# nihaomiao/CVPR23_LFDM

Measured on AMD Instinct MI355X. Metric: 40-frame 128x128 videos/sec (DDIM-100), higher is better.
Workload: dtype f32; 1 GPU; MUG 128x128, 40-frame DDIM-100 sample, batch=1 per GPU (BASELINE.json configs[1]); global_batch=1, frames=40, latent=32, image=128, sampler=DDIM-100 eta=1, cond_scale=1, parallelism=replicas x1 (videos sharded, no collective)

## Files before the change

cvpr23_lfdm_amd/csrc/attention_fused.hip:

```cpp
#include <stdlib.h>

#include "attn_core.h"
#include "../../include/lfdm_hip.h"

namespace {

#ifdef LFDM_TATTN_STAMP
struct CycleProbe {
  long long t, acc[8];
  __device__ __forceinline__ void start() {
    for (int i = 0; i < 8; ++i) acc[i] = 0;
    t = clock64();
  }
  __device__ __forceinline__ void lap(int i) {
    LFDM_SCHED_FENCE();
    const long long now = clock64();
    acc[i] += now - t;
    t = now;
    LFDM_SCHED_FENCE();
  }
};
long long* tattn_stamps = nullptr;
#define TATTN_STAMP_PARAM , long long* stamps
#define TATTN_STAMP_ARG , tattn_stamps
#else
#define TATTN_STAMP_PARAM
#define TATTN_STAMP_ARG
#endif

template <int LP, int C, bool ROT_RELOAD = false, bool WPACK = false, bool PIPE = false, bool TO_LDS = false, class PROBE = NoProbe>
__device__ __forceinline__ void tattn_heads(const float* __restrict__ x, int ldx, int head_begin, int heads_per_block,
                                            const float* __restrict__ wqkv, float* __restrict__ out, int frames, int hw, int64_t seq,
                                            const float* __restrict__ bias, const float* __restrict__ rot_cos,
                                            const float* __restrict__ rot_sin, float eps, PROBE&& probe = NoProbe{}) {
  constexpr int NT = LP / 16;
  constexpr int CQ = C / 4;

  const int lane = threadIdx.x & 63;
  const int l15 = lane & 15, lq = lane >> 4;
  const int L = frames;
  const int64_t b = seq / hw, pix = seq - b * hw;
  const int64_t row0 = b * frames * hw + pix;

  float xf[NT][CQ];
#pragma unroll
  for (int ti = 0; ti < NT; ++ti) {
    const int t = ti * 16 + l15;
    float s1 = 0.f, s2 = 0.f;
    if (t < L) {
      const float* src = x + (row0 + (int64_t)t * hw) * ldx + CQ * lq;
#pragma unroll
      for (int q = 0; q < CQ / 4; ++q) {
        const float4 v = *reinterpret_cast<const float4*>(src + 4 * q);
        xf[ti][4 * q] = v.x; xf[ti][4 * q + 1] = v.y; xf[ti][4 * q + 2] = v.z; xf[ti][4 * q + 3] = v.w;
        ln_accum(v, s1, s2);
      }
    } else {
#pragma unroll
      for (int s = 0; s < CQ; ++s) xf[ti][s] = 0.f;
    }
    float mean, rstd;
    ln_stats_slots4<false>(s1, s2, C, eps, mean, rstd);
    if (t < L) {
#pragma unroll
      for (int s = 0; s < CQ; ++s) xf[ti][s] = (xf[ti][s] - mean) * rstd;
    }
  }

  float rc[NT][4], rs[NT][4];
  if (rot_cos && !ROT_RELOAD) {
#pragma unroll
    for (int ti = 0; ti < NT; ++ti) {
      const int t = ti * 16 + l15;
      const int tt = t < L ? t : 0;
#pragma unroll
      for (int fi = 0; fi < 2; ++fi)
#pragma unroll
        for (int pr = 0; pr < 2; ++pr) {
          rc[ti][2 * fi + pr] = rot_cos[tt * 16 + 8 * fi + 2 * lq + pr];
          rs[ti][2 * fi + pr] = rot_sin[tt * 16 + 8 * fi + 2 * lq + pr];
        }
    }
  }
  const bool bias_vec = bias && (L % 4 == 0) && ((((uintptr_t)bias) & 15) == 0);
  probe.lap(4);

#pragma unroll 1
  for (int head = head_begin; head < head_begin + heads_per_block; ++head) {
    float qf[NT][8], kf[NT][8];
    {
      float wa[4][CQ];
#pragma unroll
      for (int g = 0; g < 4; ++g) {
        const float* wsrc = WPACK ? wqkv + ((int64_t)(((g >> 1) * HEADS + head) * 2 + (g & 1)) * (CQ / 4) * 64 + lane) * 4
                                  : wqkv + ((int64_t)((g >> 1) * OUT_LD + head * DH + 16 * (g & 1) + l15)) * C + CQ * lq;
#pragma unroll
        for (int q = 0; q < CQ / 4; ++q) {
          const float4 v = *reinterpret_cast<const float4*>(wsrc + (WPACK ? 256 * q : 4 * q));
          wa[g][4 * q] = v.x; wa[g][4 * q + 1] = v.y; wa[g][4 * q + 2] = v.z; wa[g][4 * q + 3] = v.w;
        }
      }
#pragma unroll
      for (int g = 0; g < 4; ++g) {
        f32x4 acc[NT];
#pragma unroll
        for (int ti = 0; ti < NT; ++ti) acc[ti] = (f32x4){0.f, 0.f, 0.f, 0.f};
#pragma unroll
        for (int s = 0; s < CQ; ++s)
#pragma unroll
          for (int ti = 0; ti < NT; ++ti) acc[ti] = mfma_16x16x4(wa[g][s], xf[ti][s], acc[ti]);
#pragma unroll
        for (int ti = 0; ti < NT; ++ti)
#pragma unroll
          for (int r = 0; r < 4; ++r) {
            if ((g >> 1) == 0) qf[ti][4 * (g & 1) + r] = acc[ti][r] * ATT_SCALE;
            else kf[ti][4 * (g & 1) + r] = acc[ti][r];
          }
      }
    }
    if (rot_cos) {
#pragma unroll
      for (int ti = 0; ti < NT; ++ti) {
#pragma unroll
        for (int fi = 0; fi < 2; ++fi)
#pragma unroll
          for (int pr = 0; pr < 2; ++pr) {
            float c, sn;
            if (ROT_RELOAD) {
              const int t = ti * 16 + l15, tt = t < L ? t : 0;
              c = rot_cos[tt * 16 + 8 * fi + 2 * lq + pr];
              sn = rot_sin[tt * 16 + 8 * fi + 2 * lq + pr];
            } else {
              c = rc[ti][2 * fi + pr];
              sn = rs[ti][2 * fi + pr];
            }
            rot_pair(qf[ti][4 * fi + 2 * pr], qf[ti][4 * fi + 2 * pr + 1], c, sn);
            rot_pair(kf[ti][4 * fi + 2 * pr], kf[ti][4 * fi + 2 * pr + 1], c, sn);
          }
      }
    }
    float vf[2][4 * NT];
    {
      float wb[2][CQ];
#pragma unroll
      for (int half = 0; half < 2; ++half) {
        const float* wsrc = WPACK ? wqkv + ((int64_t)((2 * HEADS + head) * 2 + half) * (CQ / 4) * 64 + lane) * 4
                                  : wqkv + ((int64_t)(2 * OUT_LD + head * DH + 16 * half + l15)) * C + CQ * lq;
#pragma unroll
        for (int q = 0; q < CQ / 4; ++q) {
          const float4 v = *reinterpret_cast<const float4*>(wsrc + (WPACK ? 256 * q : 4 * q));
          wb[half][4 * q] = v.x; wb[half][4 * q + 1] = v.y; wb[half][4 * q + 2] = v.z; wb[half][4 * q + 3] = v.w;
        }
      }
#pragma unroll
      for (int half = 0; half < 2; ++half) {
        f32x4 acc[NT];
#pragma unroll
        for (int ti = 0; ti < NT; ++ti) acc[ti] = (f32x4){0.f, 0.f, 0.f, 0.f};
#pragma unroll
        for (int s = 0; s < CQ; ++s)
#pragma unroll
          for (int ti = 0; ti < NT; ++ti) acc[ti] = mfma_16x16x4(xf[ti][s], wb[half][s], acc[ti]);
#pragma unroll
        for (int ti = 0; ti < NT; ++ti)
#pragma unroll
          for (int r = 0; r < 4; ++r) vf[half][4 * ti + r] = acc[ti][r];
      }
    }

    probe.lap(0);
    attend_store<NT, false, PIPE, TO_LDS>(qf, kf, vf, head, L, l15, lq, bias, bias_vec, out, row0, hw, probe);
  }
}

template <int LP, int C, bool PIPE>
__global__ __launch_bounds__(64, 2) void temporal_attn_fused_kernel(const float* __restrict__ x, int ldx, int heads_per_block,
                                                                 const float* __restrict__ wqkv,
                                                                 float* __restrict__ out, int frames, int hw,
                                                                 const float* __restrict__ bias,
                                                                 const float* __restrict__ rot_cos,
                                                                 const float* __restrict__ rot_sin, float eps) {
  tattn_heads<LP, C, false, false, PIPE>(x, ldx, blockIdx.y * heads_per_block, heads_per_block, wqkv, out, frames, hw, blockIdx.x, bias, rot_cos, rot_sin, eps);
}

template <int LP, int LROWS, int NW, bool PIPE>
__global__ __launch_bounds__(64 * NW, 2) void temporal_attn_fused_out_kernel(const float* __restrict__ x, int ldx,
                                                                          const float* __restrict__ wqkv, const float* __restrict__ wout,
                                                                          float* __restrict__ out, int ldo, int frames, int hw,
                                                                          const float* __restrict__ bias, const float* __restrict__ rot_cos,
                                                                          const float* __restrict__ rot_sin, float eps TATTN_STAMP_PARAM) {
  constexpr int C = 64, NT = LP / 16, CT = C / 16;
  __shared__ __attribute__((aligned(16))) float o_lds[LROWS * OUT_LD];
  const int wave = lfdm_uniform((int)(threadIdx.x >> 6));
  const int lane = threadIdx.x & 63, l15 = lane & 15, lq = lane >> 4;
  const int L = frames;
  const int64_t seq = blockIdx.x;
#ifdef LFDM_TATTN_STAMP
  CycleProbe probe;
  probe.start();
#else
  NoProbe probe;
#endif
  tattn_heads<LP, C, (NW < 8), true, PIPE, true>(x, ldx, wave * (HEADS / NW), HEADS / NW, wqkv, o_lds, frames, hw, seq, bias, rot_cos, rot_sin, eps, probe);
  __syncthreads();
  probe.lap(5);
  const int64_t b = seq / hw, pix = seq - b * hw;
  const int64_t row0 = b * frames * hw + pix;
  for (int tile = wave; tile < NT * CT; tile += NW) {
    const int ti = tile / CT, ct = tile - ti * CT;
    const int t = ti * 16 + l15;
    const int tr = t < L ? t : L - 1;
    const float* arow = o_lds + tr * OUT_LD;
    const float* brow = wout + ((int64_t)ct * (OUT_LD / 16) * 64 + lane) * 4;
    f32x4 acc = {0.f, 0.f, 0.f, 0.f}, acc1 = acc;
    float xr[4];
#pragma unroll
    for (int r = 0; r < 4; ++r) {
      const int tok = ti * 16 + 4 * lq + r;
      xr[r] = x[(row0 + (int64_t)(tok < L ? tok : L - 1) * hw) * ldx + ct * 16 + l15];
    }
#pragma unroll 4
    for (int S = 0; S < OUT_LD / 16; S += 2) {
      const float4 a = *reinterpret_cast<const float4*>(arow + (((4 * S + lq) ^ (tr & 15)) << 2));
      const float4 a1 = *reinterpret_cast<const float4*>(arow + (((4 * S + 4 + lq) ^ (tr & 15)) << 2));
      const float4 w = *reinterpret_cast<const float4*>(brow + 256 * S);
      const float4 w1 = *reinterpret_cast<const float4*>(brow + 256 * S + 256);
      acc = mfma_16x16x4(a.x, w.x, acc);
      acc1 = mfma_16x16x4(a1.x, w1.x, acc1);
      acc = mfma_16x16x4(a.y, w.y, acc);
      acc1 = mfma_16x16x4(a1.y, w1.y, acc1);
      acc = mfma_16x16x4(a.z, w.z, acc);
      acc1 = mfma_16x16x4(a1.z, w1.z, acc1);
      acc = mfma_16x16x4(a.w, w.w, acc);
      acc1 = mfma_16x16x4(a1.w, w1.w, acc1);
    }
#pragma unroll
    for (int r = 0; r < 4; ++r) acc[r] += acc1[r];
#pragma unroll
    for (int r = 0; r < 4; ++r) {
      const int tok = ti * 16 + 4 * lq + r;
      if (tok < L) {
        const int64_t row = row0 + (int64_t)tok * hw;
        out[row * ldo + ct * 16 + l15] = acc[r] + xr[r];
      }
    }
  }
#ifdef LFDM_TATTN_STAMP
  probe.lap(6);
  if (stamps && lane == 0 && blockIdx.x < 256)
    for (int i = 0; i < 8; ++i) stamps[((int64_t)blockIdx.x * 8 + wave) * 8 + i] = probe.acc[i];
#endif
}

template <int LP, bool PIPE>
__global__ __launch_bounds__(64, 1) void temporal_attn_fused_wide_kernel(const float* __restrict__ x, int ldx, int channels,
                                                                      int heads_per_block, const float* __restrict__ wqkv,
                                                                      float* __restrict__ out, int frames, int hw,
                                                                      const float* __restrict__ bias,
                                                                      const float* __restrict__ rot_cos,
                                                                      const float* __restrict__ rot_sin, float eps) {
  constexpr int NT = LP / 16;
  const int lane = threadIdx.x & 63;
  const int l15 = lane & 15, lq = lane >> 4;
  const int L = frames;
  const int64_t seq = blockIdx.x;
  const int64_t b = seq / hw, pix = seq - b * hw;
  const int64_t row0 = b * frames * hw + pix;
  const int ncb = channels / 64;

  float mean[NT], rstd[NT];
#pragma unroll
  for (int ti = 0; ti < NT; ++ti) {
    const int t = ti * 16 + l15;
    float s1 = 0.f, s2 = 0.f;
    if (t < L) {
      const float* src = x + (row0 + (int64_t)t * hw) * ldx + 16 * lq;
      for (int cb = 0; cb < ncb; ++cb)
#pragma unroll
        for (int q = 0; q < 4; ++q) ln_accum(*reinterpret_cast<const float4*>(src + 64 * cb + 4 * q), s1, s2);
    }
    ln_stats_slots4<true>(s1, s2, channels, eps, mean[ti], rstd[ti]);
  }
  const bool bias_vec = bias && (L % 4 == 0) && ((((uintptr_t)bias) & 15) == 0);

  const int head_begin = blockIdx.y * heads_per_block;
#pragma unroll 1
  for (int head = head_begin; head < head_begin + heads_per_block; ++head) {
    f32x4 aq[2][NT], ak[2][NT], av[2][NT];
#pragma unroll
    for (int g = 0; g < 2; ++g)
#pragma unroll
      for (int ti = 0; ti < NT; ++ti) aq[g][ti] = ak[g][ti] = av[g][ti] = (f32x4){0.f, 0.f, 0.f, 0.f};
#pragma unroll 1
    for (int cb = 0; cb < ncb; ++cb) {
      float w[6][16];
#pragma unroll
      for (int g = 0; g < 6; ++g) {
        const float* wsrc = wqkv + ((int64_t)((g >> 1) * OUT_LD + head * DH + 16 * (g & 1) + l15)) * channels + 64 * cb + 16 * lq;
#pragma unroll
        for (int q = 0; q < 4; ++q) {
          const float4 v = *reinterpret_cast<const float4*>(wsrc + 4 * q);
          w[g][4 * q] = v.x; w[g][4 * q + 1] = v.y; w[g][4 * q + 2] = v.z; w[g][4 * q + 3] = v.w;
        }
      }
#pragma unroll
      for (int ti = 0; ti < NT; ++ti) {
        const int t = ti * 16 + l15;
        float xf[16];
        if (t < L) {
          const float* src = x + (row0 + (int64_t)t * hw) * ldx + 64 * cb + 16 * lq;
#pragma unroll
          for (int q = 0; q < 4; ++q) {
            const float4 v = *reinterpret_cast<const float4*>(src + 4 * q);
            xf[4 * q] = (v.x - mean[ti]) * rstd[ti]; xf[4 * q + 1] = (v.y - mean[ti]) * rstd[ti];
            xf[4 * q + 2] = (v.z - mean[ti]) * rstd[ti]; xf[4 * q + 3] = (v.w - mean[ti]) * rstd[ti];
          }
        } else {
#pragma unroll
          for (int s2 = 0; s2 < 16; ++s2) xf[s2] = 0.f;
        }
#pragma unroll
        for (int s2 = 0; s2 < 16; ++s2) {
          aq[0][ti] = mfma_16x16x4(w[0][s2], xf[s2], aq[0][ti]);
          aq[1][ti] = mfma_16x16x4(w[1][s2], xf[s2], aq[1][ti]);
          ak[0][ti] = mfma_16x16x4(w[2][s2], xf[s2], ak[0][ti]);
          ak[1][ti] = mfma_16x16x4(w[3][s2], xf[s2], ak[1][ti]);
          av[0][ti] = mfma_16x16x4(xf[s2], w[4][s2], av[0][ti]);
          av[1][ti] = mfma_16x16x4(xf[s2], w[5][s2], av[1][ti]);
        }
      }
    }
    float qf[NT][8], kf[NT][8], vf[2][4 * NT];
#pragma unroll
    for (int ti = 0; ti < NT; ++ti)
#pragma unroll
      for (int fi = 0; fi < 2; ++fi)
#pragma unroll
        for (int r = 0; r < 4; ++r) {
          qf[ti][4 * fi + r] = aq[fi][ti][r] * ATT_SCALE;
          kf[ti][4 * fi + r] = ak[fi][ti][r];
          vf[fi][4 * ti + r] = av[fi][ti][r];
        }
    if (rot_cos) {
#pragma unroll
      for (int ti = 0; ti < NT; ++ti) {
        const int t = ti * 16 + l15;
        const int tt = t < L ? t : 0;
#pragma unroll
        for (int fi = 0; fi < 2; ++fi)
#pragma unroll
          for (int pr = 0; pr < 2; ++pr) {
            const float c = rot_cos[tt * 16 + 8 * fi + 2 * lq + pr], sn = rot_sin[tt * 16 + 8 * fi + 2 * lq + pr];
            rot_pair(qf[ti][4 * fi + 2 * pr], qf[ti][4 * fi + 2 * pr + 1], c, sn);
            rot_pair(kf[ti][4 * fi + 2 * pr], kf[ti][4 * fi + 2 * pr + 1], c, sn);
          }
      }
    }
    attend_store<NT, false, PIPE>(qf, kf, vf, head, L, l15, lq, bias, bias_vec, out, row0, hw);
  }
}

int launch_fused_wide(const float* x, int ldx, int channels, const float* wqkv, float* out, int batch, int frames, int hw,
                      const float* bias, const float* rot_cos, const float* rot_sin, float eps, hipStream_t stream) {
  const int64_t nseq = (int64_t)batch * hw;
  int hpb = 8;
  while (hpb > 1 && nseq * (HEADS / hpb) < 2048) hpb >>= 1;
  const dim3 grid((unsigned)nseq, (unsigned)(HEADS / hpb)), block(64);
  lp_ladder(frames, [&](auto lp) {
    constexpr int LP = decltype(lp)::value;
    if (bias_by_quads(bias, frames))
      LFDM_LAUNCH((temporal_attn_fused_wide_kernel<LP, true>), grid, block, 0, stream, x, ldx, channels, hpb, wqkv, out, frames, hw, bias, rot_cos, rot_sin, eps);
    else
      LFDM_LAUNCH((temporal_attn_fused_wide_kernel<LP, false>), grid, block, 0, stream, x, ldx, channels, hpb, wqkv, out, frames, hw, bias, rot_cos, rot_sin, eps);
  });
  return lfdm_check_launch("temporal_attention_fused_wide");
}

template <int C>
int launch_fused(const float* x, int ldx, const float* wqkv, float* out, int batch, int frames, int hw, const float* bias,
                 const float* rot_cos, const float* rot_sin, float eps, hipStream_t stream) {
  const int64_t nseq = (int64_t)batch * hw;
  int hpb = 8;
  while (hpb > 1 && nseq * (HEADS / hpb) < 2048) hpb >>= 1;
  if (const char* e = lfdm_knob("LFDM_TATTN_HPB")) {
    const int v = atoi(e);
    if (v == 1 || v == 2 || v == 4 || v == 8) hpb = v;
  }
  const dim3 grid((unsigned)nseq, (unsigned)(HEADS / hpb)), block(64);
  lp_ladder(frames, [&](auto lp) {
    constexpr int LP = decltype(lp)::value;
    constexpr bool CAN_PIPE = LP <= 32;
    if (CAN_PIPE && bias_by_quads(bias, frames))
      LFDM_LAUNCH((temporal_attn_fused_kernel<LP, C, CAN_PIPE>), grid, block, 0, stream, x, ldx, hpb, wqkv, out, frames, hw, bias, rot_cos, rot_sin, eps);
    else
      LFDM_LAUNCH((temporal_attn_fused_kernel<LP, C, false>), grid, block, 0, stream, x, ldx, hpb, wqkv, out, frames, hw, bias, rot_cos, rot_sin, eps);
  });
  return lfdm_check_launch("temporal_attention_fused");
}

template <int LP, int LROWS>
int launch_fused_out_lp(const float* x, int ldx, const float* wqkv, const float* wout, float* out, int ldo, int batch, int frames, int hw,
                        const float* bias, const float* rot_cos, const float* rot_sin, float eps, hipStream_t stream) {
  const int64_t nseq = (int64_t)batch * hw;
  int nw = 2;
  while (nw < 8 && nseq * nw < 2048) nw <<= 1;
  if (const char* e = getenv("LFDM_TATTN_OUT_NW")) {
    const int v = atoi(e);
    if (v == 1 || v == 2 || v == 4 || v == 8) nw = v;
  }
  const dim3 grid((unsigned)nseq);
  lfdm_ladder<1, 2, 4, 8>(nw, [&](auto nwc) {
    constexpr int NW = decltype(nwc)::value;
#if defined(LFDM_TATTN_STAMP) && LFDM_TATTN_STAMP == 2
    constexpr bool CAN_PIPE = false;
#else
    constexpr bool CAN_PIPE = !(LP == 64 && NW == 4);
#endif
    if (CAN_PIPE && bias_by_quads(bias, frames))
      LFDM_LAUNCH((temporal_attn_fused_out_kernel<LP, LROWS, NW, CAN_PIPE>), grid, dim3(64 * NW), 0, stream, x, ldx, wqkv, wout, out, ldo, frames, hw, bias, rot_cos, rot_sin, eps TATTN_STAMP_ARG);
    else
      LFDM_LAUNCH((temporal_attn_fused_out_kernel<LP, LROWS, NW, false>), grid, dim3(64 * NW), 0, stream, x, ldx, wqkv, wout, out, ldo, frames, hw, bias, rot_cos, rot_sin, eps TATTN_STAMP_ARG);
  });
  return lfdm_check_launch("temporal_attention_fused_out");
}

}

#ifdef LFDM_TATTN_STAMP
extern "C" void lfdm_tattn_stamp_buffer(void* p) { tattn_stamps = (long long*)p; }
#endif

extern "C" int lfdm_temporal_attention_fused_out_cl_f32(const float* x, int ldx, int channels, const float* wqkv, const float* wout,
                                                        float* out, int ldo, int batch, int frames, int hw, const float* bias,
                                                        const float* rot_cos, const float* rot_sin, float ln_eps, lfdm_stream_t stream_) {
  hipStream_t stream = (hipStream_t)stream_;
  if (!x || !wqkv || !wout || !out || batch <= 0 || frames <= 0 || frames > 64 || hw <= 0 || channels != 64 || ldx < 64 || ldx % 4 != 0 ||
      ldo < 64 || (((uintptr_t)x | (uintptr_t)wqkv | (uintptr_t)wout) & 15) || ((rot_cos == nullptr) != (rot_sin == nullptr)) || out == x) {
    lfdm_set_error("temporal_attention_fused_out: needs C == 64, frames <= 64, 16-byte aligned rows, out != x");
    return LFDM_EINVAL;
  }
  return lp_ladder(frames, [&](auto lp) {
    constexpr int LP = decltype(lp)::value;
    if (LP == 48 && frames <= 40)
      return launch_fused_out_lp<48, 40>(x, ldx, wqkv, wout, out, ldo, batch, frames, hw, bias, rot_cos, rot_sin, ln_eps, stream);
    return launch_fused_out_lp<LP, LP>(x, ldx, wqkv, wout, out, ldo, batch, frames, hw, bias, rot_cos, rot_sin, ln_eps, stream);
  });
}

extern "C" int lfdm_temporal_attention_fused_cl_f32(const float* x, int ldx, int channels, const float* wqkv, float* out,
                                                    int batch, int frames, int hw, const float* bias,
                                                    const float* rot_cos, const float* rot_sin, float ln_eps,
                                                    lfdm_stream_t stream_) {
  hipStream_t stream = (hipStream_t)stream_;
  if (!x || !wqkv || !out || batch <= 0 || frames <= 0 || frames > 64 || hw <= 0 || ldx < channels || ldx % 4 != 0 ||
      (((uintptr_t)x | (uintptr_t)wqkv) & 15) || ((rot_cos == nullptr) != (rot_sin == nullptr)) ||
      channels < 64 || channels % 64 != 0) {
    lfdm_set_error("temporal_attention_fused: needs C % 64 == 0, frames <= 64, 16-byte aligned rows");
    return LFDM_EINVAL;
  }
  if (channels == 64) return launch_fused<64>(x, ldx, wqkv, out, batch, frames, hw, bias, rot_cos, rot_sin, ln_eps, stream);
  return launch_fused_wide(x, ldx, channels, wqkv, out, batch, frames, hw, bias, rot_cos, rot_sin, ln_eps, stream);
}
```

cvpr23_lfdm_amd/csrc/lfdm_device.h:

```cpp
#pragma once
#include <stddef.h>
#include <stdint.h>
#include <type_traits>

#if defined(LFDM_EMU_BUILD)
#include "hip_emu.h"
typedef emu_f32x16 f32x16;
typedef emu_f32x4 f32x4;
#define LFDM_LAUNCH(kern, grid, block, smem, stream, ...) \
  emu::launch(grid, block, smem, [=]() { kern(__VA_ARGS__); })
static inline f32x16 mfma_32x32x2(float a, float b, f32x16 c) { return emu_mfma_32x32x2(a, b, c); }
static inline f32x4 mfma_16x16x4(float a, float b, f32x4 c) { return emu_mfma_16x16x4(a, b, c); }
static inline f32x4 mfma_4x4x1(float a, float b, f32x4 c) { return emu_mfma_4x4x1(a, b, c); }
struct lfdm_bf16x8 { uint16_t h[8]; };
static inline uint16_t lfdm_f32_to_bf16(float f) {
  uint32_t u;
  memcpy(&u, &f, 4);
  if ((u & 0x7fffffffu) > 0x7f800000u) return (uint16_t)((u >> 16) | 0x40u);
  u += 0x7fffu + ((u >> 16) & 1u);
  return (uint16_t)(u >> 16);
}
static inline float lfdm_bf16_to_f32(uint16_t h) {
  const uint32_t u = (uint32_t)h << 16;
  float f;
  memcpy(&f, &u, 4);
  return f;
}
static inline lfdm_bf16x8 lfdm_cvt_bf16x8(float4 a0, float4 a1) {
  const float f[8] = {a0.x, a0.y, a0.z, a0.w, a1.x, a1.y, a1.z, a1.w};
  lfdm_bf16x8 r;
  for (int i = 0; i < 8; ++i) r.h[i] = lfdm_f32_to_bf16(f[i]);
  return r;
}
static inline uint32_t lfdm_cvt_pk_bf16(float lo, float hi) { return (uint32_t)lfdm_f32_to_bf16(lo) | ((uint32_t)lfdm_f32_to_bf16(hi) << 16); }
static inline lfdm_bf16x8 lfdm_bf16x8_bits(float4 v) {
  lfdm_bf16x8 r;
  memcpy(&r, &v, 16);
  return r;
}
static inline f32x16 mfma_32x32x16_bf16(lfdm_bf16x8 a, lfdm_bf16x8 b, f32x16 c) {
  struct Pair { lfdm_bf16x8 a, b; };
  struct Whole { lfdm_bf16x8 a[2], b[2]; };
  const unsigned lane = emu::lane_id(), h = lane >> 5;
  const Pair other = emu::wave_read_from(Pair{a, b}, lane ^ 32u);
  Whole mine;
  mine.a[h] = a;
  mine.a[1 - h] = other.a;
  mine.b[h] = b;
  mine.b[1 - h] = other.b;
  for (int r = 0; r < 16; ++r) {
    const unsigned row = (r & 3) + 8 * (r >> 2) + 4 * h;
    const Whole src = emu::wave_read_from(mine, row);
    float acc = c[r];
    for (int k = 0; k < 16; ++k)
      acc = fmaf(lfdm_bf16_to_f32(src.a[k >> 3].h[k & 7]), lfdm_bf16_to_f32(mine.b[k >> 3].h[k & 7]), acc);
    c[r] = acc;
  }
  return c;
}
#else
#include <hip/hip_runtime.h>
typedef float f32x16 __attribute__((ext_vector_type(16)));
typedef float f32x4 __attribute__((ext_vector_type(4)));
#define LFDM_LAUNCH(kern, grid, block, smem, stream, ...) \
  hipLaunchKernelGGL(kern, grid, block, smem, stream, __VA_ARGS__)
__device__ __forceinline__ f32x16 mfma_32x32x2(float a, float b, f32x16 c) {
  return __builtin_amdgcn_mfma_f32_32x32x2f32(a, b, c, 0, 0, 0);
}
__device__ __forceinline__ f32x4 mfma_16x16x4(float a, float b, f32x4 c) {
  return __builtin_amdgcn_mfma_f32_16x16x4f32(a, b, c, 0, 0, 0);
}
__device__ __forceinline__ f32x4 mfma_4x4x1(float a, float b, f32x4 c) {
  return __builtin_amdgcn_mfma_f32_4x4x1f32(a, b, c, 0, 0, 0);
}
typedef __bf16 lfdm_bf16x8 __attribute__((ext_vector_type(8)));
typedef __bf16 lfdm_bf16x2 __attribute__((ext_vector_type(2)));
typedef float lfdm_f32x8 __attribute__((ext_vector_type(8)));
typedef float lfdm_f32x2 __attribute__((ext_vector_type(2)));
__device__ __forceinline__ lfdm_bf16x8 lfdm_cvt_bf16x8(float4 a0, float4 a1) {
  const lfdm_f32x8 f = {a0.x, a0.y, a0.z, a0.w, a1.x, a1.y, a1.z, a1.w};
  return __builtin_convertvector(f, lfdm_bf16x8);
}
__device__ __forceinline__ uint32_t lfdm_cvt_pk_bf16(float lo, float hi) {
  const lfdm_f32x2 f = {lo, hi};
  return __builtin_bit_cast(uint32_t, __builtin_convertvector(f, lfdm_bf16x2));
}
__device__ __forceinline__ lfdm_bf16x8 lfdm_bf16x8_bits(float4 v) { return __builtin_bit_cast(lfdm_bf16x8, v); }
__device__ __forceinline__ f32x16 mfma_32x32x16_bf16(lfdm_bf16x8 a, lfdm_bf16x8 b, f32x16 c) {
  return __builtin_amdgcn_mfma_f32_32x32x16_bf16(a, b, c, 0, 0, 0);
}
#endif

#define LFDM_WAVE 64

template <int BEGIN, int END, class F>
__device__ __forceinline__ void lfdm_static_for(F&& f) {
  if constexpr (BEGIN < END) {
    f(std::integral_constant<int, BEGIN>{});
    lfdm_static_for<BEGIN + 1, END>(f);
  }
}

template <int R, int... REST, class F>
inline auto lfdm_ladder(int v, F&& f) {
  if constexpr (sizeof...(REST) == 0) return f(std::integral_constant<int, R>{});
  else return v <= R ? f(std::integral_constant<int, R>{}) : lfdm_ladder<REST...>(v, f);
}

#if defined(LFDM_EMU_BUILD)
struct lfdm_buf {
  const char* base;
  uint32_t bytes;
};
static inline lfdm_buf lfdm_make_buf(const void* p, uint32_t bytes) { return lfdm_buf{(const char*)p, bytes}; }
static inline float4 lfdm_buf_load_f4(lfdm_buf b, uint32_t off) {
  float4 v = make_float4(0.f, 0.f, 0.f, 0.f);
  if ((uint64_t)off + 16u <= (uint64_t)b.bytes) memcpy(&v, b.base + off, 16);
  return v;
}
static inline float2 lfdm_buf_load_f2(lfdm_buf b, uint32_t off) {
  float2 v = make_float2(0.f, 0.f);
  if ((uint64_t)off + 8u <= (uint64_t)b.bytes) memcpy(&v, b.base + off, 8);
  return v;
}
#else
typedef __amdgpu_buffer_rsrc_t lfdm_buf;
typedef int lfdm_i32x4 __attribute__((ext_vector_type(4)));
__device__ __forceinline__ lfdm_buf lfdm_make_buf(const void* p, uint32_t bytes) {
  return __builtin_amdgcn_make_buffer_rsrc(const_cast<void*>(p), 0, (int)bytes, 0x00020000);
}
__device__ __forceinline__ float4 lfdm_buf_load_f4(lfdm_buf b, uint32_t off) {
  const lfdm_i32x4 v = __builtin_amdgcn_raw_buffer_load_b128(b, (int)off, 0, 0);
  float4 f;
  f.x = __int_as_float(v.x);
  f.y = __int_as_float(v.y);
  f.z = __int_as_float(v.z);
  f.w = __int_as_float(v.w);
  return f;
}
typedef int lfdm_i32x2 __attribute__((ext_vector_type(2)));
__device__ __forceinline__ float2 lfdm_buf_load_f2(lfdm_buf b, uint32_t off) {
  const lfdm_i32x2 v = __builtin_amdgcn_raw_buffer_load_b64(b, (int)off, 0, 0);
  return make_float2(__int_as_float(v.x), __int_as_float(v.y));
}
#endif
#define LFDM_BUF_OOB 0xFFFFFFF0u

#if defined(LFDM_EMU_BUILD)
static inline void lfdm_buf_store_f4_sc1(lfdm_buf b, uint32_t off, float4 v) {
  if ((uint64_t)off + 16u <= (uint64_t)b.bytes) memcpy(const_cast<char*>(b.base) + off, &v, 16);
}
static inline float4 lfdm_buf_load_f4_sc1(lfdm_buf b, uint32_t off) { return lfdm_buf_load_f4(b, off); }
#else
__device__ __forceinline__ void lfdm_buf_store_f4_sc1(lfdm_buf b, uint32_t off, float4 v) {
  lfdm_i32x4 d;
  d.x = __float_as_int(v.x); d.y = __float_as_int(v.y); d.z = __float_as_int(v.z); d.w = __float_as_int(v.w);
  __builtin_amdgcn_raw_buffer_store_b128(d, b, (int)off, 0, 16);
}
__device__ __forceinline__ float4 lfdm_buf_load_f4_sc1(lfdm_buf b, uint32_t off) {
  const lfdm_i32x4 v = __builtin_amdgcn_raw_buffer_load_b128(b, (int)off, 0, 16);
  float4 f;
  f.x = __int_as_float(v.x); f.y = __int_as_float(v.y); f.z = __int_as_float(v.z); f.w = __int_as_float(v.w);
  return f;
}
#endif

#if defined(LFDM_EMU_BUILD)
template <int OFF = 0> static inline void lfdm_gload_f4(f32x4& dst, const float* p) { memcpy(&dst, (const char*)p + OFF, 16); }
template <int N> static inline void lfdm_vmwait() {}
template <int N> static inline void lfdm_vmwait(f32x4&) {}
template <int N> static inline void lfdm_vmwait(f32x4&, f32x4&) {}
template <int N> static inline void lfdm_vmwait(f32x4&, f32x4&, f32x4&, f32x4&) {}
static inline void lfdm_tie(f32x4&) {}
static inline int lfdm_uniform(int v) { return v; }
#else
template <int OFF = 0>
__device__ __forceinline__ void lfdm_gload_f4(f32x4& dst, const float* p) {
  asm volatile("global_load_dwordx4 %0, %1, off offset:%2" : "=v"(dst) : "v"(p), "n"(OFF) : "memory");
}
template <int N> __device__ __forceinline__ void lfdm_vmwait() { asm volatile("s_waitcnt vmcnt(%0)" ::"n"(N) : "memory"); }
template <int N> __device__ __forceinline__ void lfdm_vmwait(f32x4& a) { asm volatile("s_waitcnt vmcnt(%1)" : "+v"(a) : "n"(N) : "memory"); }
template <int N> __device__ __forceinline__ void lfdm_vmwait(f32x4& a, f32x4& b) {
  asm volatile("s_waitcnt vmcnt(%2)" : "+v"(a), "+v"(b) : "n"(N) : "memory");
}
template <int N> __device__ __forceinline__ void lfdm_vmwait(f32x4& a, f32x4& b, f32x4& c, f32x4& d) {
  asm volatile("s_waitcnt vmcnt(%4)" : "+v"(a), "+v"(b), "+v"(c), "+v"(d) : "n"(N) : "memory");
}
__device__ __forceinline__ void lfdm_tie(f32x4& a) { asm volatile("" : "+v"(a)::"memory"); }
__device__ __forceinline__ int lfdm_uniform(int v) { return __builtin_amdgcn_readfirstlane(v); }
#endif

#if defined(LFDM_EMU_BUILD)
#define LFDM_DRAIN_STORES() ((void)0)
#define LFDM_FENCE_RELEASE_AGENT() ((void)0)
#define LFDM_FENCE_ACQUIRE_AGENT() ((void)0)
static inline unsigned lfdm_ticket_take(unsigned* c) { return __atomic_fetch_add(c, 1u, __ATOMIC_SEQ_CST); }
static inline void lfdm_ticket_reset(unsigned* c) { __atomic_store_n(c, 0u, __ATOMIC_SEQ_CST); }
#else
#define LFDM_DRAIN_STORES() asm volatile("s_waitcnt vmcnt(0)" ::: "memory")
#define LFDM_FENCE_RELEASE_AGENT() __builtin_amdgcn_fence(__ATOMIC_RELEASE, "agent")
#define LFDM_FENCE_ACQUIRE_AGENT() __builtin_amdgcn_fence(__ATOMIC_ACQUIRE, "agent")
__device__ __forceinline__ unsigned lfdm_ticket_take(unsigned* c) {
  return __hip_atomic_fetch_add(c, 1u, __ATOMIC_RELAXED, __HIP_MEMORY_SCOPE_AGENT);
}
__device__ __forceinline__ void lfdm_ticket_reset(unsigned* c) {
  __hip_atomic_store(c, 0u, __ATOMIC_RELAXED, __HIP_MEMORY_SCOPE_AGENT);
}
#endif

#if defined(__HIP_DEVICE_COMPILE__) && !defined(__gfx950__) && !defined(LFDM_EMU_BUILD)
#error "fence-free hand-off (lfdm_agent_store_u64 / lfdm_agent_load_u64 / lfdm_ticket_take) validated on gfx950 only: re-validate, or use LFDM_FENCE_RELEASE_AGENT / LFDM_FENCE_ACQUIRE_AGENT, before building for another target"
#endif
#if defined(LFDM_EMU_BUILD)
static inline void lfdm_agent_store_u64(unsigned long long* p, unsigned long long v) { __atomic_store_n(p, v, __ATOMIC_SEQ_CST); }
static inline unsigned long long lfdm_agent_load_u64(const unsigned long long* p) { return __atomic_load_n(p, __ATOMIC_SEQ_CST); }
static inline unsigned lfdm_agent_load_u32(const unsigned* p) { return __atomic_load_n(p, __ATOMIC_SEQ_CST); }
static inline void lfdm_sleep() {}
#else
__device__ __forceinline__ void lfdm_agent_store_u64(unsigned long long* p, unsigned long long v) {
  __hip_atomic_store(p, v, __ATOMIC_RELAXED, __HIP_MEMORY_SCOPE_AGENT);
}
__device__ __forceinline__ unsigned long long lfdm_agent_load_u64(const unsigned long long* p) {
  return __hip_atomic_load(p, __ATOMIC_RELAXED, __HIP_MEMORY_SCOPE_AGENT);
}
__device__ __forceinline__ unsigned lfdm_agent_load_u32(const unsigned* p) { return __hip_atomic_load(p, __ATOMIC_RELAXED, __HIP_MEMORY_SCOPE_AGENT); }
__device__ __forceinline__ void lfdm_sleep() { __builtin_amdgcn_s_sleep(2); }
#endif

#if defined(LFDM_EMU_BUILD)
#define LFDM_SCHED_FENCE() ((void)0)
#define LFDM_SCHED_GROUP(mask, n) ((void)0)
#else
#define LFDM_SCHED_FENCE() __builtin_amdgcn_sched_barrier(0)
#define LFDM_SCHED_GROUP(mask, n) __builtin_amdgcn_sched_group_barrier(mask, n, 0)
#endif
#define LFDM_SG_VALU 0x002
#define LFDM_SG_MFMA 0x008

#if defined(LFDM_EMU_BUILD)
static inline void lfdm_wave_lds_sync() { emu::wave_sync(); }
#else
__device__ __forceinline__ void lfdm_wave_lds_sync() {
  __builtin_amdgcn_fence(__ATOMIC_RELEASE, "wavefront");
  __builtin_amdgcn_wave_barrier();
  __builtin_amdgcn_fence(__ATOMIC_ACQUIRE, "wavefront");
}
#endif

__device__ __forceinline__ float wave_sum(float v) {
#pragma unroll
  for (int m = 32; m >= 1; m >>= 1) v += __shfl_xor(v, m);
  return v;
}
__device__ __forceinline__ float wave_max(float v) {
#pragma unroll
  for (int m = 32; m >= 1; m >>= 1) v = fmaxf(v, __shfl_xor(v, m));
  return v;
}
#if defined(LFDM_EMU_BUILD)
static inline float fast_exp(float x) { return expf(x); }
static inline float fast_rcp(float x) { return 1.0f / x; }
#else
__device__ __forceinline__ float fast_exp(float x) { return __expf(x); }
__device__ __forceinline__ float fast_rcp(float x) { return __builtin_amdgcn_rcpf(x); }
#endif
__device__ __forceinline__ float sigmoidf_(float x) { return 1.0f / (1.0f + expf(-x)); }
__device__ __forceinline__ float siluf_(float x) { return x / (1.0f + expf(-x)); }

#if defined(LFDM_EMU_BUILD)
static inline float silu_fast_(float x) { return x / (1.0f + expf(-x)); }
#else
__device__ __forceinline__ float silu_fast_(float x) { return x * __builtin_amdgcn_rcpf(1.0f + __expf(-x)); }
#endif

#if defined(LFDM_TUNING_KNOBS) || defined(LFDM_EMU_BUILD)
static inline const char* lfdm_knob(const char* name) { return getenv(name); }
#else
static inline const char* lfdm_knob(const char*) { return nullptr; }
#endif

__device__ __forceinline__ float apply_act(float v, int act) {
  if (act == 1) return v > 0.f ? v : 0.f;
  if (act == 2) return sigmoidf_(v);
  if (act == 3) return siluf_(v);
  return v;
}

extern "C" void lfdm_set_error(const char* msg);
int lfdm_check_launch(const char* what);
```

Before: 4.180 videos/s.

## Restructure temporal attention out-projection with register weight ring and column-major wave mapping

The output projection in the fused temporal attention kernel is rewritten so each wave owns fixed output column tiles and handles several token tiles at once. The wout fragments are prefetched into a register ring before the barrier, overlapping global loads with the attention tail. LDS A-operands are double-buffered across steps. This reuses weights across token tiles and hides load latency, at the cost of higher register pressure that may hurt occupancy. Lane id is recomputed through mbcnt to keep it out of long-lived registers.

Result: no change. 4.201 videos/s (median of 6 runs) (+0.5%).

```diff
diff --git a/cvpr23_lfdm_amd/csrc/attention_fused.hip b/cvpr23_lfdm_amd/csrc/attention_fused.hip
--- a/cvpr23_lfdm_amd/csrc/attention_fused.hip
+++ b/cvpr23_lfdm_amd/csrc/attention_fused.hip
@@ -183,6 +183,94 @@
   tattn_heads<LP, C, false, false, PIPE>(x, ldx, blockIdx.y * heads_per_block, heads_per_block, wqkv, out, frames, hw, blockIdx.x, bias, rot_cos, rot_sin, eps);
 }
 
+template <int WD>
+__device__ __forceinline__ float4 wout_fragment(const float* __restrict__ wout, int ct0, int ctstep, int p, int lane) {
+  const float* frag = wout + (int64_t)((ct0 + (p >> 4) * ctstep) * (OUT_LD / 16) + (p & 15)) * 256;
+  return *reinterpret_cast<const float4*>(frag + 4 * lane);
+}
+template <int WD>
+__device__ __forceinline__ void wout_ring_fill(float4 (&w)[WD], const float* __restrict__ wout, int ct0, int ctstep, int lane) {
+#pragma unroll
+  for (int p = 0; p < WD; ++p) w[p] = wout_fragment<WD>(wout, ct0, ctstep, p, lane);
+}
+
+template <int M, int NCT, int WD>
+__device__ __forceinline__ void to_out_columns(float4 (&w)[WD], const float* o_lds, const float* __restrict__ wout,
+                                               const float* __restrict__ x, int ldx, float* __restrict__ out, int ldo, int ct0, int ctstep,
+                                               int ti0, int tstep, int L, int64_t row0, int hw, int lane) {
+  constexpr int NS = OUT_LD / 16;
+  const int l15 = lane & 15, lq = lane >> 4;
+  const float* aq[M][4];
+#pragma unroll
+  for (int m = 0; m < M; ++m) {
+    const int t = (ti0 + m * tstep) * 16 + l15;
+    const int tr = t < L ? t : L - 1;
+#pragma unroll
+    for (int j = 0; j < 4; ++j) aq[m][j] = o_lds + tr * OUT_LD + (((4 * j + lq) ^ (tr & 15)) << 2);
+  }
+  float4 a[2][M], a1[2][M];
+#pragma unroll
+  for (int m = 0; m < M; ++m) {
+    a[0][m] = *reinterpret_cast<const float4*>(aq[m][0]);
+    a1[0][m] = *reinterpret_cast<const float4*>(aq[m][1]);
+  }
+#pragma unroll
+  for (int i = 0; i < NCT; ++i) {
+    const int ct = ct0 + i * ctstep;
+    float xr[M][4];
+#pragma unroll
+    for (int m = 0; m < M; ++m)
+#pragma unroll
+      for (int r = 0; r < 4; ++r) {
+        const int tok = (ti0 + m * tstep) * 16 + 4 * lq + r;
+        xr[m][r] = x[(row0 + (int64_t)(tok < L ? tok : L - 1) * hw) * ldx + ct * 16 + l15];
+      }
+    f32x4 acc[M], acc1[M];
+#pragma unroll
+    for (int m = 0; m < M; ++m) acc[m] = acc1[m] = (f32x4){0.f, 0.f, 0.f, 0.f};
+#pragma unroll
+    for (int S = 0; S < NS; S += 2) {
+      constexpr int HS = NS / 2;
+      const int step = i * HS + S / 2, cur = step & 1, p = i * NS + S;
+      if (step + 1 < NCT * HS) {
+        const int Sn = (S + 2) % NS;
+#pragma unroll
+        for (int m = 0; m < M; ++m) {
+          a[cur ^ 1][m] = *reinterpret_cast<const float4*>(aq[m][Sn & 3] + 64 * (Sn >> 2));
+          a1[cur ^ 1][m] = *reinterpret_cast<const float4*>(aq[m][(Sn + 1) & 3] + 64 * (Sn >> 2));
+        }
+      }
+      const float4 w0 = w[p % WD], w1 = w[(p + 1) % WD];
+#pragma unroll
+      for (int m = 0; m < M; ++m) { acc[m] = mfma_16x16x4(a[cur][m].x, w0.x, acc[m]); acc1[m] = mfma_16x16x4(a1[cur][m].x, w1.x, acc1[m]); }
+#pragma unroll
+      for (int m = 0; m < M; ++m) { acc[m] = mfma_16x16x4(a[cur][m].y, w0.y, acc[m]); acc1[m] = mfma_16x16x4(a1[cur][m].y, w1.y, acc1[m]); }
+#pragma unroll
+      for (int m = 0; m < M; ++m) { acc[m] = mfma_16x16x4(a[cur][m].z, w0.z, acc[m]); acc1[m] = mfma_16x16x4(a1[cur][m].z, w1.z, acc1[m]); }
+#pragma unroll
+      for (int m = 0; m < M; ++m) { acc[m] = mfma_16x16x4(a[cur][m].w, w0.w, acc[m]); acc1[m] = mfma_16x16x4(a1[cur][m].w, w1.w, acc1[m]); }
+      if (p + WD < NCT * NS) {
+        w[p % WD] = wout_fragment<WD>(wout, ct0, ctstep, p + WD, lane);
+        w[(p + 1) % WD] = wout_fragment<WD>(wout, ct0, ctstep, p + WD + 1, lane);
+      }
+      LFDM_SCHED_FENCE();
+    }
+#pragma unroll
+    for (int m = 0; m < M; ++m) {
+#pragma unroll
+      for (int r = 0; r < 4; ++r) acc[m][r] += acc1[m][r];
+#pragma unroll
+      for (int r = 0; r < 4; ++r) {
+        const int tok = (ti0 + m * tstep) * 16 + 4 * lq + r;
+        if (tok < L) {
+          const int64_t row = row0 + (int64_t)tok * hw;
+          out[row * ldo + ct * 16 + l15] = acc[m][r] + xr[m][r];
+        }
+      }
+    }
+  }
+}
+
 template <int LP, int LROWS, int NW, bool PIPE>
 __global__ __launch_bounds__(64 * NW, 2) void temporal_attn_fused_out_kernel(const float* __restrict__ x, int ldx,
                                                                           const float* __restrict__ wqkv, const float* __restrict__ wout,
@@ -192,7 +280,6 @@
   constexpr int C = 64, NT = LP / 16, CT = C / 16;
   __shared__ __attribute__((aligned(16))) float o_lds[LROWS * OUT_LD];
   const int wave = lfdm_uniform((int)(threadIdx.x >> 6));
-  const int lane = threadIdx.x & 63, l15 = lane & 15, lq = lane >> 4;
   const int L = frames;
   const int64_t seq = blockIdx.x;
 #ifdef LFDM_TATTN_STAMP
@@ -202,49 +289,21 @@
   NoProbe probe;
 #endif
   tattn_heads<LP, C, (NW < 8), true, PIPE, true>(x, ldx, wave * (HEADS / NW), HEADS / NW, wqkv, o_lds, frames, hw, seq, bias, rot_cos, rot_sin, eps, probe);
+  constexpr int NCT = NW >= CT ? 1 : CT / NW;
+  constexpr int RS = NW > CT ? NW / CT : 1;
+  constexpr int MT = (NT + RS - 1) / RS;
+  const int ct0 = RS > 1 ? wave % CT : wave, h = RS > 1 ? wave / CT : 0;
+  const bool whole = h + (MT - 1) * RS < NT;
+  constexpr int WD = LP == 16 ? 4 : OUT_LD / 16;
+  float4 wring[WD];
+  const int lane = lfdm_lane_again();
+  if (MT > 1 || whole) wout_ring_fill<WD>(wring, wout, ct0, NW, lane);
   __syncthreads();
   probe.lap(5);
   const int64_t b = seq / hw, pix = seq - b * hw;
   const int64_t row0 = b * frames * hw + pix;
-  for (int tile = wave; tile < NT * CT; tile += NW) {
-    const int ti = tile / CT, ct = tile - ti * CT;
-    const int t = ti * 16 + l15;
-    const int tr = t < L ? t : L - 1;
-    const float* arow = o_lds + tr * OUT_LD;
-    const float* brow = wout + ((int64_t)ct * (OUT_LD / 16) * 64 + lane) * 4;
-    f32x4 acc = {0.f, 0.f, 0.f, 0.f}, acc1 = acc;
-    float xr[4];
-#pragma unroll
-    for (int r = 0; r < 4; ++r) {
-      const int tok = ti * 16 + 4 * lq + r;
-      xr[r] = x[(row0 + (int64_t)(tok < L ? tok : L - 1) * hw) * ldx + ct * 16 + l15];
-    }
-#pragma unroll 4
-    for (int S = 0; S < OUT_LD / 16; S += 2) {
-      const float4 a = *reinterpret_cast<const float4*>(arow + (((4 * S + lq) ^ (tr & 15)) << 2));
-      const float4 a1 = *reinterpret_cast<const float4*>(arow + (((4 * S + 4 + lq) ^ (tr & 15)) << 2));
-      const float4 w = *reinterpret_cast<const float4*>(brow + 256 * S);
-      const float4 w1 = *reinterpret_cast<const float4*>(brow + 256 * S + 256);
-      acc = mfma_16x16x4(a.x, w.x, acc);
-      acc1 = mfma_16x16x4(a1.x, w1.x, acc1);
-      acc = mfma_16x16x4(a.y, w.y, acc);
-      acc1 = mfma_16x16x4(a1.y, w1.y, acc1);
-      acc = mfma_16x16x4(a.z, w.z, acc);
-      acc1 = mfma_16x16x4(a1.z, w1.z, acc1);
-      acc = mfma_16x16x4(a.w, w.w, acc);
-      acc1 = mfma_16x16x4(a1.w, w1.w, acc1);
-    }
-#pragma unroll
-    for (int r = 0; r < 4; ++r) acc[r] += acc1[r];
-#pragma unroll
-    for (int r = 0; r < 4; ++r) {
-      const int tok = ti * 16 + 4 * lq + r;
-      if (tok < L) {
-        const int64_t row = row0 + (int64_t)tok * hw;
-        out[row * ldo + ct * 16 + l15] = acc[r] + xr[r];
-      }
-    }
-  }
+  if (whole) to_out_columns<MT, NCT, WD>(wring, o_lds, wout, x, ldx, out, ldo, ct0, NW, h, RS, L, row0, hw, lane);
+  else if (MT > 1) to_out_columns<(MT > 1 ? MT - 1 : 1), NCT, WD>(wring, o_lds, wout, x, ldx, out, ldo, ct0, NW, h, RS, L, row0, hw, lane);
 #ifdef LFDM_TATTN_STAMP
   probe.lap(6);
   if (stamps && lane == 0 && blockIdx.x < 256)
diff --git a/cvpr23_lfdm_amd/csrc/lfdm_device.h b/cvpr23_lfdm_amd/csrc/lfdm_device.h
--- a/cvpr23_lfdm_amd/csrc/lfdm_device.h
+++ b/cvpr23_lfdm_amd/csrc/lfdm_device.h
@@ -173,6 +173,7 @@
 template <int N> static inline void lfdm_vmwait(f32x4&, f32x4&, f32x4&, f32x4&) {}
 static inline void lfdm_tie(f32x4&) {}
 static inline int lfdm_uniform(int v) { return v; }
+static inline int lfdm_lane_again() { return (int)(threadIdx.x & 63); }
 #else
 template <int OFF = 0>
 __device__ __forceinline__ void lfdm_gload_f4(f32x4& dst, const float* p) {
@@ -188,6 +189,11 @@
 }
 __device__ __forceinline__ void lfdm_tie(f32x4& a) { asm volatile("" : "+v"(a)::"memory"); }
 __device__ __forceinline__ int lfdm_uniform(int v) { return __builtin_amdgcn_readfirstlane(v); }
+__device__ __forceinline__ int lfdm_lane_again() {
+  unsigned z;
+  asm volatile("s_mov_b32 %0, 0" : "=s"(z));
+  return (int)__builtin_amdgcn_mbcnt_hi(~0u, __builtin_amdgcn_mbcnt_lo(~0u, z));
+}
 #endif
 
 #if defined(LFDM_EMU_BUILD)
```
